# Ycblue/TransMIL-DeepGraft

Measured on AMD Instinct MI355X. Metric: slides/sec (fwd+bwd) at N=8192 patches, d=512, higher is better.
Workload: dtype bf16; 1 GPU; TransMIL_feat 2-class, 1 bag N=8192x512 per GPU, train step fwd+CE+bwd+allreduce+Lookahead(RAdam); execution=hipGraph replay of the whole step (one graph per resident bag), global_batch=1, seq_len=8192, parallelism=dp1, accumulate_grad_batches=1

## Files before the change

### include/transmil_hip.h

```cpp
#ifndef TRANSMIL_HIP_H
#define TRANSMIL_HIP_H
#include <stdint.h>

#ifdef __cplusplus
extern "C" {
#endif

const char* tm_last_error(void);
const char* tm_build_info(void);

enum { TM_EPI_PLAIN = 0, TM_EPI_QKV = 1, TM_EPI_SPLITK = 2 };
typedef struct tm_gemm_args {
  int M, N, K;
  int lda, ldb, ldc;
  int a_trans, b_kn;
  int ab_dtype, c_dtype;
  int splits, k_per_split;
  int mode;
  float alpha;
  const float* bias;
  int gelu;
  void* pre;
  int ld_pre;
  float drop_p, drop_scale;
  uint64_t seed;
  const float* resid;
  int accumulate;
  int grp_in, skip, grp_out, out_off, dup_n, dup_off;
  int nbags, nh, dh, seq;
  float qscale;
  const uint64_t* seed_ptr;
  float* colsum;
  int pre_bf16;
  int slab_bf16;
} tm_gemm_args;

int tm_gemm(const void* A, const void* B, void* C, const tm_gemm_args* args, void* stream);
typedef struct tm_reduce_queue tm_reduce_queue;
tm_reduce_queue* tm_reduce_queue_create(void);
void tm_reduce_queue_destroy(tm_reduce_queue* rq);
int tm_reduce_queue_pending(const tm_reduce_queue* rq);
int tm_reduce_flush(tm_reduce_queue* rq, void* stream);
int tm_splitk_reduce(const float* slab, float* out, int splits, long long count, float alpha,
                     int accumulate, tm_reduce_queue* rq, void* stream);
int tm_splitk_reduce_bf16(const void* slab, float* out, int splits, long long count, float alpha,
                          int accumulate, tm_reduce_queue* rq, void* stream);
long long tm_colsum_workspace(int rows, int cols, int rows_per_chunk);
int tm_colsum(const void* X, int dtype, int rows, int cols, int ld, int rows_per_chunk,
              float* work, float* out, int accumulate, tm_reduce_queue* rq, void* stream);

int tm_layernorm_fwd(const float* x, const float* gamma, const float* beta, float eps, int rows, int D,
                     int S, int n_pad, int pad, int dtype, void* y, float* mean, float* rstd, void* stream);
long long tm_layernorm_bwd_workspace(int rows, int D, int rows_per_block);
int tm_layernorm_bwd(const void* dy, int dtype, const float* x, const float* gamma, const float* mean,
                     const float* rstd, int rows, int D, int S, int n_pad, int pad, int rows_per_block,
                     int resid_cls_only, float* dx_accum, float* work, float* dgamma, float* dbeta,
                     tm_reduce_queue* rq, void* stream);
int tm_layernorm_bwd_seg(const void* dy, int dtype, const float* x, const float* gamma, const float* mean,
                         const float* rstd, int rows, int D, int S, int n_pad, int pad, int rows_per_block,
                         int resid_cls_only, const float* seg_add, int seg_len, int nseg, int seg_rows,
                         float* dx_accum, float* work, float* dgamma, float* dbeta, tm_reduce_queue* rq,
                         void* stream);
int tm_head_fwd(const float* h, int B, int S, int D, const float* gamma, const float* beta, float eps,
                const float* W, const float* bias, int C, float* logits, float* xhat, float* rstd,
                void* stream);
int tm_head_bwd(const float* dlogits, int B, int C, int S, int D, const float* xhat, const float* rstd,
                const float* gamma, const float* beta, const float* W, float* dW, float* dbias,
                float* dgamma, float* dbeta, float* dh, void* stream);
int tm_head_ce_fwd(const float* h, int B, int S, int D, const float* gamma, const float* beta, float eps,
                   const float* W, const float* bias, int C, const long long* label, float* logits, float* xhat,
// ... 258 lines not shown
```

### transmil_deepgraft_amd/_lib.py

```python
from __future__ import annotations

import ctypes as C
import os

_HERE = os.path.dirname(os.path.abspath(__file__))
LIB_PATH = os.environ.get("TRANSMIL_HIP_LIB", os.path.join(_HERE, "libtransmil_hip.so"))

F32, BF16 = 0, 1
EPI_PLAIN, EPI_QKV, EPI_SPLITK = 0, 1, 2

P = C.c_void_p
I = C.c_int
L = C.c_longlong
Fl = C.c_float
U64 = C.c_uint64


class GemmArgs(C.Structure):
    _fields_ = [("M", I), ("N", I), ("K", I), ("lda", I), ("ldb", I), ("ldc", I),
                ("a_trans", I), ("b_kn", I), ("ab_dtype", I), ("c_dtype", I),
                ("splits", I), ("k_per_split", I), ("mode", I), ("alpha", Fl),
                ("bias", P), ("gelu", I), ("pre", P), ("ld_pre", I),
                ("drop_p", Fl), ("drop_scale", Fl), ("seed", U64), ("resid", P),
                ("accumulate", I), ("grp_in", I), ("skip", I), ("grp_out", I),
# ... 4 lines not shown
class BmmJob(C.Structure):
    _fields_ = [("A", P), ("B", P), ("ta", I), ("tb", I), ("lda", I), ("ldb", I), ("sa", L), ("sb", L),
                ("A2", P), ("B2", P), ("ta2", I), ("tb2", I), ("lda2", I), ("ldb2", I), ("sa2", L), ("sb2", L),
                ("E1", P), ("e1", Fl), ("E2", P), ("e2", Fl), ("alpha", Fl), ("diag", Fl),
                ("C", P), ("ldc", I), ("sc", L), ("M", I), ("N", I), ("K", I),
                ("C2", P), ("c2_alpha", Fl), ("c2_diag", Fl), ("c2_e1", Fl),
                ("Ct", P), ("ct_plane", L), ("ct_mode", I), ("ct_reserved", I), ("Rd", P), ("Rw", P)]


OPTIM_MAX_TENSORS = 40


class OptimTensor(C.Structure):
    _fields_ = [("param", P), ("grad", P), ("numel", L), ("lr", Fl), ("weight_decay", Fl)]


class OptimTable(C.Structure):
    _fields_ = [("count", I), ("reserved", I), ("offset", L * (OPTIM_MAX_TENSORS + 1)),
                ("t", OptimTensor * OPTIM_MAX_TENSORS), ("hyper", P)]


CAST_MAX = 8


class CastTable(C.Structure):
    _fields_ = [("count", I), ("reserved", I), ("src", P * CAST_MAX), ("dst", P * CAST_MAX),
                ("offset", L * (CAST_MAX + 1))]


_SIGS = {
    "tm_last_error": (C.c_char_p, []),
    "tm_build_info": (C.c_char_p, []),
    "tm_gemm": (I, [P, P, P, C.POINTER(GemmArgs), P]),
    "tm_splitk_reduce": (I, [P, P, I, L, Fl, I, P, P]),
    "tm_splitk_reduce_bf16": (I, [P, P, I, L, Fl, I, P, P]),
    "tm_colsum_workspace": (L, [I, I, I]),
    "tm_colsum": (I, [P, I, I, I, I, I, P, P, I, P, P]),
    "tm_layernorm_fwd": (I, [P, P, P, Fl, I, I, I, I, I, I, P, P, P, P]),
    "tm_layernorm_bwd_workspace": (L, [I, I, I]),
    "tm_layernorm_bwd": (I, [P, I, P, P, P, P, I, I, I, I, I, I, I, P, P, P, P, P, P]),
    "tm_layernorm_bwd_seg": (I, [P, I, P, P, P, P, I, I, I, I, I, I, I, P, I, I, I, P, P, P, P, P, P]),
    "tm_head_fwd": (I, [P, I, I, I, P, P, Fl, P, P, I, P, P, P, P]),
    "tm_head_bwd": (I, [P, I, I, I, I, P, P, P, P, P, P, P, P, P, P, P]),
    "tm_head_ce_fwd": (I, [P, I, I, I, P, P, Fl, P, P, I, P, P, P, P, P, P, P, P, P]),
    "tm_head_ce_bwd": (I, [P, P, P, P, I, I, I, I, P, P, P, P, P, P, P, P, P, P, P, P]),
    "tm_nys_landmarks": (I, [I, P, P, I, I, P, P, P, P, P]),
    "tm_nys_sim2_softmax": (I, [P, P, I, P, P]),
    "tm_softmax_bwd_rows256": (I, [P, P, P, I, P]),
    "tm_nys_a3_workspace": (L, [I, I]),
    "tm_nys_a3_partials": (L, [I, I]),
    "tm_nys_a3_fwd": (I, [I, P, P, P, I, I, P, P, P, P]),
    "tm_nys_a3_fwd_sim2": (I, [P, P, P, P, I, I, P, P, P, P]),
    "tm_nys_a1_fwd": (I, [I, P, P, P, P, P, I, I, I, P, P, P]),
    "tm_cast_f32": (I, [I, P, P, L, P]),
    "tm_nys_conv_bwd_workspace": (L, [I, I, I]),
    "tm_nys_conv_bwd": (I, [I, P, P, P, P, I, I, I, P, P, P, P, P, P]),
    "tm_nys_a1_bwd_workspace": (L, [I, I, I]),
    "tm_nys_a1_bwd": (I, [I, P, P, P, P, P, P, I, I, I, I, P, P, P, P, I, P, P]),
    "tm_nys_a1_bwd_dqkv": (I, [P, P, P, P, P, P, I, I, I, P, Fl, P, P, P, P, P]),
    "tm_nys_a3_bwd_workspace": (L, [I, I]),
    "tm_nys_a3_bwd": (I, [I, P, P, P, P, P, P, I, I, I, P, P, P, P, I, P, P]),
    "tm_nys_assemble_dqkv": (I, [I, P, P, P, P, P, I, I, I, Fl, P, P]),
    "tm_nys_a3_bwd_fused": (I, [P, P, P, P, P, P, I, I, I, P, I, I, P, P, P, P, P, P]),
    "tm_nys_a3_bwd_slabs": (I, [I, I]),
    "tm_nys_assemble_q_slab": (I, [I, P, I, P, P, I, I, I, I, Fl, P, P]),
    "tm_nys_assemble_q_slab_inplace": (I, [P, P, I, I, I, I, Fl, P, P]),
# ... 143 lines not shown
```

### transmil_deepgraft_amd/csrc/gemm.hip

```cpp
#include <new>

#include "common.h"

#include <type_traits>
#include "../../include/transmil_hip.h"

namespace {

constexpr int BM = 128, BN = 128;
constexpr int EP_ROW = BN + 8;

template <typename T> struct Tile {
  static constexpr int E = 16 / sizeof(T);
  static constexpr int BK = 128 / sizeof(T);
  static constexpr int KROW = BK + E;
  static constexpr int TROW = BM + 32;
  static constexpr int KSTEPS = BK / 16;
  static constexpr int CHUNKS = BM * BK / E / 256;
};

template <typename T> union Chunk { f32x4 raw; T e[16 / sizeof(T)]; };

template <typename T>
TM_DEV void load_rows_full(Chunk<T> (&st)[Tile<T>::CHUNKS], const T* X, int ld, int r0, int k0, int tid) {
// ... 509 lines not shown
  auto mm = [](f32x16& c, const bf16x8& a, const bf16x8& b) { mma16(c, a, b); };
  bf16x8 a[2], b[2][2];
  rd_frag<A_KS, 0>(a[0], abase, akc); rd_frag<B_KS, 0>(b[0][0], b0, bkc0); rd_frag<B_KS, 0>(b[0][1], b1, bkc1);
  rd_frag<A_KS, 1>(a[1], abase, akc); rd_frag<B_KS, 1>(b[1][0], b0, bkc0); rd_frag<B_KS, 1>(b[1][1], b1, bkc1);
  wait_lgkm<RS>();
  mm(acc[0], a[0], b[0][0]);
  mm(acc[1], a[0], b[0][1]);
  rd_frag<A_KS, 2>(a[0], abase, akc); rd_frag<B_KS, 2>(b[0][0], b0, bkc0); rd_frag<B_KS, 2>(b[0][1], b1, bkc1);
  wait_lgkm<RS>();
  mm(acc[0], a[1], b[1][0]);
  mm(acc[1], a[1], b[1][1]);
  rd_frag<A_KS, 3>(a[1], abase, akc); rd_frag<B_KS, 3>(b[1][0], b0, bkc0); rd_frag<B_KS, 3>(b[1][1], b1, bkc1);
  wait_lgkm<RS>();
  mm(acc[0], a[0], b[0][0]);
  mm(acc[1], a[0], b[0][1]);
  wait_lgkm<0>();
  mm(acc[0], a[1], b[1][0]);
  mm(acc[1], a[1], b[1][1]);
}

__device__ unsigned long long g_gemm_stamps[2048 * 8];
template <bool ON>
TM_DEV void ring_stamp(unsigned long long (&ts)[8], int slot, bool real = false) {
  if constexpr (ON) {
    __builtin_amdgcn_sched_barrier(0);
    unsigned long long t;
    if (real) asm volatile("s_memrealtime %0\n\ts_waitcnt lgkmcnt(0)" : "=s"(t)::"memory");
    else asm volatile("s_memtime %0\n\ts_waitcnt lgkmcnt(0)" : "=s"(t)::"memory");
    __builtin_amdgcn_sched_barrier(0);
    ts[slot] = t;
  }
}

template <typename OutT, bool A_T, bool B_KN, bool STAMP = false, int KIND = EK_ANY>
__global__ __launch_bounds__(512) __attribute__((amdgpu_waves_per_eu(4))) void gemm_ring_kernel(const bf16* __restrict__ A, const bf16* __restrict__ B,
                                                        OutT* __restrict__ C, tm_gemm_args g) {
  extern __shared__ __attribute__((aligned(16))) char smem[];
  unsigned long long ts[8] = {0, 0, 0, 0, 0, 0, 0, 0};
  ring_stamp<STAMP>(ts, 0, true);
  ring_stamp<STAMP>(ts, 1);
  const int tid = threadIdx.x, lane = tid & 63;
  const int wave = __builtin_amdgcn_readfirstlane(tid >> 6);
  const int wm = wave >> 1, wn = wave & 1;
  int m0, n0, zs;
  tile_split_of_block(m0, n0, zs);
  const int kbeg = zs * g.k_per_split;
  const int kend = min(g.K, kbeg + g.k_per_split);
  const int nk = kend > kbeg ? (kend - kbeg) / 64 : 0;

  f32x16 acc[2];
  acc[0] = (f32x16){};
  acc[1] = (f32x16){};
  constexpr bool COLSUM = A_T && KIND == EK_SPLITK && !STAMP;
  const bool do_cs = COLSUM && g.colsum != nullptr && n0 == 0;
  const int cs_c = tid & 15, cs_r = tid >> 4;
  float csum[8] = {0.f, 0.f, 0.f, 0.f, 0.f, 0.f, 0.f, 0.f};
  unsigned akc[4] = {0, 0, 0, 0}, bkc0[4] = {0, 0, 0, 0}, bkc1[4] = {0, 0, 0, 0};
  unsigned aks = 0, bks0 = 0, bks1 = 0;
  if constexpr (A_T) aks = ks_addr(wm * 32, lane); else kc_addrs(akc, wm * 32, lane);
  if constexpr (B_KN) {
    bks0 = ks_addr(wn * 64, lane) + STAGE_BYTES / 2;
    bks1 = ks_addr(wn * 64 + 32, lane) + STAGE_BYTES / 2;
  } else {
    kc_addrs(bkc0, wn * 64, lane);
    kc_addrs(bkc1, wn * 64 + 32, lane);
#pragma unroll
    for (int s = 0; s < 4; ++s) { bkc0[s] += STAGE_BYTES / 2; bkc1[s] += STAGE_BYTES / 2; }
  }
  const unsigned ring = lds_u32(smem);

  auto issue = [&](int kt) {
    char* st = smem + (kt % NSTAGE) * STAGE_BYTES;
    const int k0 = kbeg + kt * 64;
    glds_tile<A_T>(st, A, g.lda, m0, g.M, k0, wave, lane);
    glds_tile<B_KN>(st + STAGE_BYTES / 2, B, g.ldb, n0, g.N, k0, wave, lane);
  };
#pragma unroll
  for (int t = 0; t < NSTAGE - 1; ++t)
// ... 34 lines not shown
    if (do_cs) {
#pragma unroll
      for (int e = 0; e < 8; ++e) {
        csum[e] += __shfl_xor(csum[e], 16, 64);
        csum[e] += __shfl_xor(csum[e], 32, 64);
      }
      __syncthreads();
      float* red = (float*)smem;
      if (lane < 16) {
#pragma unroll
        for (int e = 0; e < 8; ++e) red[wave * 128 + cs_c * 8 + e] = csum[e];
      }
      __syncthreads();
      if (tid < 128 && m0 + tid < g.M) {
        float s = 0.f;
#pragma unroll
        for (int w = 0; w < 8; ++w) s += red[w * 128 + tid];
        g.colsum[(size_t)zs * g.M + m0 + tid] = s;
      }
    }
  }
  if constexpr (STAMP) {
    ring_stamp<STAMP>(ts, 5);
    asm volatile("s_waitcnt vmcnt(0)" ::: "memory");
    ring_stamp<STAMP>(ts, 6);
    ring_stamp<STAMP>(ts, 7, true);
    const int blk = (blockIdx.z * gridDim.y + blockIdx.y) * gridDim.x + blockIdx.x;
    if (tid < 8 && blk < 2048) {
      unsigned long long v = ts[0];
#pragma unroll
      for (int i = 1; i < 8; ++i) v = tid == i ? ts[i] : v;
      g_gemm_stamps[blk * 8 + tid] = v;
    }
  }
}

constexpr int BM160 = 160;
constexpr int R160_A = BM160 * 128, R160_STAGE = R160_A + 128 * 128;

TM_DEV void tile160_of_block(int& m0, int& n0) {
  const int ntx = gridDim.x, nwg = gridDim.x * gridDim.y;
  const int orig = blockIdx.y * ntx + blockIdx.x;
  const int q = nwg / 8, r = nwg % 8, xcd = orig % 8;
  const int id = (xcd < r ? xcd * (q + 1) : r * (q + 1) + (xcd - r) * q) + orig / 8;
  m0 = (id / ntx) * BM160;
  n0 = (id % ntx) * BN;
}

template <typename OutT, bool B_KN, int KIND = EK_ANY>
__global__ __launch_bounds__(640) void gemm_ring160_kernel(const bf16* __restrict__ A, const bf16* __restrict__ B,
                                                           OutT* __restrict__ C, tm_gemm_args g) {
  extern __shared__ __attribute__((aligned(16))) char smem[];
  typedef __attribute__((address_space(3))) void lds_t;
  typedef __attribute__((address_space(1))) void glb_t;
  const int tid = threadIdx.x, lane = tid & 63;
  const int wave = __builtin_amdgcn_readfirstlane(tid >> 6);
  const int wm = wave >> 1, wn = wave & 1;
  int m0, n0;
  tile160_of_block(m0, n0);
  const int nk = g.K / 64;

  f32x16 acc[2];
  acc[0] = (f32x16){};
  acc[1] = (f32x16){};
  unsigned akc[4], bkc0[4] = {0, 0, 0, 0}, bkc1[4] = {0, 0, 0, 0};
  unsigned bks0 = 0, bks1 = 0;
// ... 385 lines not shown
      float t = slab[i];
      for (int z = 1; z < splits; ++z) t += slab[(size_t)z * count + i];
      t *= alpha;
      if (accumulate) t += out[i];
      out[i] = t;
    }
  }
}

template <typename T>
__global__ void colsum_partial_kernel(const T* __restrict__ X, int rows, int cols, int ld, int rows_per_chunk,
                                      float* __restrict__ part) {
  const int c = blockIdx.x * 64 + (threadIdx.x & 63);
  const int sub = threadIdx.x >> 6;
  const int r0 = blockIdx.y * rows_per_chunk, r1 = min(rows, r0 + rows_per_chunk);
  __shared__ float red[4][64];
  float s = 0.f;
  if (c < cols) {
    float p8[8] = {0.f, 0.f, 0.f, 0.f, 0.f, 0.f, 0.f, 0.f};
    int r = r0 + sub;
    for (; r + 28 < r1; r += 32) {
#pragma unroll
      for (int j = 0; j < 8; ++j) p8[j] += to_f(X[(size_t)(r + 4 * j) * ld + c]);
    }
    for (; r < r1; r += 4) p8[0] += to_f(X[(size_t)r * ld + c]);
    s = ((p8[0] + p8[1]) + (p8[2] + p8[3])) + ((p8[4] + p8[5]) + (p8[6] + p8[7]));
  }
  red[sub][threadIdx.x & 63] = s;
  __syncthreads();
  if (sub == 0 && c < cols)
    part[(size_t)blockIdx.y * cols + c] = red[0][threadIdx.x] + red[1][threadIdx.x] + red[2][threadIdx.x] + red[3][threadIdx.x];
}

}

extern "C" int tm_gemm(const void* A, const void* B, void* C, const tm_gemm_args* g, void* stream) {
  TM_REQUIRE(g && A && B && C, "gemm: null argument");
  TM_REQUIRE(g->M >= 0 && g->N >= 0 && g->K >= 0 && g->splits >= 1, "gemm: bad shape");
  TM_REQUIRE(g->mode != TM_EPI_SPLITK || g->c_dtype == TM_F32, "gemm: split-K slabs are fp32 (or bf16 via slab_bf16)");
  TM_REQUIRE(!g->slab_bf16 || (g->mode == TM_EPI_SPLITK && g->ab_dtype == TM_BF16),
             "gemm: slab_bf16 is for bf16 split-K weight gradients");
  TM_REQUIRE(g->k_per_split > 0, "gemm: k_per_split must be > 0");
  TM_REQUIRE(((uintptr_t)A % 16) == 0 && ((uintptr_t)B % 16) == 0, "gemm: operands must be 16-B aligned");
  const int E = g->ab_dtype == TM_BF16 ? 8 : 4;
  TM_REQUIRE(g->lda % E == 0 && g->ldb % E == 0, "gemm: leading dimensions must be multiples of 16 B");
  TM_REQUIRE(g->mode != TM_EPI_QKV || (g->dh % 8 == 0 && g->N % 8 == 0), "gemm: QKV scatter needs dh % 8 == 0");
  if (g->M == 0 || g->N == 0) return 0;
  TM_REQUIRE(!g->colsum || (g->ab_dtype == TM_BF16 && g->c_dtype == TM_F32 && g->a_trans && g->mode == TM_EPI_SPLITK &&
                            pick_path(*g) == PATH_RING && GEMM_SEL != GEMM_STAMP_RING),
             "gemm: colsum needs the bf16 split-K weight-gradient ring path (a_trans, K % 64 == 0, M % 8 == 0)");
  hipStream_t st = (hipStream_t)stream;
  if (g->ab_dtype == TM_BF16) {
    TM_REQUIRE(g->k_per_split % 64 == 0 || g->splits == 1, "gemm: bf16 k_per_split must be a multiple of 64");
    if (g->c_dtype == TM_BF16) return launch_t<bf16, bf16>(A, B, C, *g, st);
    return launch_t<bf16, float>(A, B, C, *g, st);
  }
  TM_REQUIRE(g->ab_dtype == TM_F32, "gemm: ab_dtype");
  TM_REQUIRE(g->k_per_split % 32 == 0 || g->splits == 1, "gemm: f32 k_per_split must be a multiple of 32");
  if (g->c_dtype == TM_BF16) return launch_t<float, bf16>(A, B, C, *g, st);
  return launch_t<float, float>(A, B, C, *g, st);
}

#ifdef TM_DIAG
extern "C" void tm_debug_set_gemm_sel(int sel) { g_gemm_sel = sel; }

extern "C" int tm_debug_gemm_stamps(unsigned long long* host, int count) {
  TM_REQUIRE(count > 0 && count <= 2048 * 8, "gemm_stamps: bad count");
  if (hipMemcpyFromSymbol(host, HIP_SYMBOL(g_gemm_stamps), count * sizeof(unsigned long long)) != hipSuccess) {
    tm_set_error("gemm_stamps: copy");
    return 1;
  }
  return 0;
}
#endif

namespace {
constexpr int DEFER_MAX = 48;
struct ReduceEntry {
  const void* slab;
  float* out;
  long long count;
  int splits;
  int accumulate;
  float alpha;
  int vec;
  int par;
  int bf16;
};
struct ReduceTable {
  ReduceEntry e[DEFER_MAX];
  long long off[DEFER_MAX + 1];
  int boff[DEFER_MAX + 1];
  int n;
// ... 229 lines not shown
```

### transmil_deepgraft_amd/engine.py

```python
from __future__ import annotations

import ctypes as C
import math
from dataclasses import dataclass

import torch

from . import _lib
from ._lib import BF16, F32, EPI_PLAIN, EPI_QKV, EPI_SPLITK, GemmArgs, BmmJob

NL = 256
DH = 64
TAPS = 33
PINV_ITERS = 6
LN_EPS = 1e-5
GEOMETRIES = ((DH, NL), (32, 128), (48, 192))
QROWS = NL + 32
CLS_Q_ROWS = True


class _Probe:

    def __init__(self):
        self.target = None
# ... 245 lines not shown
    def __exit__(self, *exc):
        try:
            if exc[0] is None and self.q.pending() > 0:
                self.q.flush()
        finally:
            _TLS.queue = self.prev
            self.q.close()
        return False


def _rq():
    q = getattr(_TLS, "queue", None)
    if q is not None and getattr(_TLS, "deferring", False):
        return q.handle
    return C.c_void_p(0)


class defer_reductions:

    def __enter__(self):
        self.prev = getattr(_TLS, "deferring", False)
        _TLS.deferring = getattr(_TLS, "queue", None) is not None
        return self

    def __exit__(self, *exc):
        _TLS.deferring = self.prev
        return False


def flush_reductions():
    q = getattr(_TLS, "queue", None)
    if q is not None:
        q.flush()


def nystrom_core_forward(qkv, geo: Geometry, wconv, tdtype, dt_code, pool, cls_row=None):
    if (geo.dh, geo.nl) != (DH, NL):
        if cls_row is not None:
            raise NotImplementedError("the class-row layer runs at dim_head=64, num_landmarks=256 only")
        return _nysg_core_forward(qkv, geo, wconv, pool)
    n, nbh, nh = geo.n, geo.nbh, geo.heads
    q, k, v = qkv[0], qkv[1], qkv[2]
    st = _stream()
    ql = pool(nbh * NL * DH).view(nbh, NL, DH)
    kl = pool(nbh * NL * DH).view(nbh, NL, DH)
    ql_t = pool(nbh * NL * DH, tdtype).view(nbh, NL, DH)
    kl_t = pool(nbh * NL * DH, tdtype).view(nbh, NL, DH)
    with probe("landmarks"):
        _lib.call("tm_nys_landmarks", dt_code, _p(q), _p(k), nbh, n, _p(ql), _p(kl), _p(ql_t), _p(kl_t), st)
    a2 = pool(nbh * NL * NL).view(nbh, NL, NL)
    w = pool(nbh * NL * DH).view(nbh, NL, DH)
    lse3 = pool(nbh * NL)
    work = pool(_lib.query("tm_nys_a3_workspace", nbh, n) // 4)
    prec = 1 if dt_code == BF16 else 0
    a2s = None
    if prec:
        a2s = pool(nbh * NL * NL)
        with probe("a3_fwd"):
            _lib.call("tm_nys_a3_fwd_sim2", _p(ql), _p(kl), _p(k), _p(v), nbh, n, _p(work), _p(a2), _p(a2s), st)
    else:
        with probe("a3_fwd"):
            _lib.call("tm_nys_a3_fwd", dt_code, _p(ql), _p(k), _p(v), nbh, n, _p(work), _p(w), _p(lse3), st)
    if prec:
        saved = pool(_lib.query("tm_pinv_split_saved_floats", nbh, PINV_ITERS))
        with probe("pinv_fwd"):
            _lib.call("tm_pinv_fwd_split_a3", _p(a2), _p(a2s), nbh, PINV_ITERS, _p(saved), _p(work),
# ... 220 lines not shown
    _lib.call("tm_nysg_assemble_dqkv", dh, nl, dt_code, _p(dq), _p(dql), _p(dk), _p(dkl), _p(dv), geo.B, nh, n,
              C.c_float(scale), _p(dqkv), st)
    return dqkv


def translayer_forward(H, geo: Geometry, prm, tdtype, dt_code, pool, drop_p, seed, seed_dev=None, cls_only=False):
    B, S, n, D, pad = geo.B, geo.S, geo.n, geo.D, geo.pad
    st = _stream()
    xn = pool(B * n * D, tdtype).view(B, n, D)
    mean = pool(B * S)
    rstd = pool(B * S)
    with probe("ln_fwd"):
        _lib.call("tm_layernorm_fwd", _p(H), _p(prm["norm_w"]), _p(prm["norm_b"]), C.c_float(LN_EPS), B * S, D,
                  S, n, pad, dt_code, _p(xn), _p(mean), _p(rstd), st)
    qkv = pool(3 * geo.nbh * n * DH, tdtype).view(3, geo.nbh, n, DH)
    with probe("qkv_gemm"):
        gemm(xn, prm["wqkv"], qkv, B * n, 3 * D, D, lda=D, ldb=D, ldc=0, dtype=dt_code,
             qkv=(B, geo.heads, DH, n, DH ** -0.5))
    merged, state = nystrom_core_forward(qkv, geo, prm["wconv"], tdtype, dt_code, pool,
                                         cls_row=pad if cls_only else None)
    Hout = pool(B * S * D).view(B * S, D)
    if cls_only:
        _lib.call("tm_cls_out_fwd", dt_code, _p(merged), _p(prm["wo"]), _p(prm["bo"]), _p(H), B, n, pad, S, D,
                  C.c_float(drop_p), C.c_uint64(seed), _p(seed_dev), _p(Hout), st)
    else:
        with probe("out_gemm"):
            gemm(merged, prm["wo"], Hout, B * n, D, D, lda=D, ldb=D, ldc=D, dtype=dt_code, c_dtype=F32,
                 bias=prm["bo"], drop_p=drop_p, seed=seed, seed_ptr=seed_dev, resid=H, rowmap=(n, pad, S, 0, 0, 0))
    saved = dict(xn=xn, mean=mean, rstd=rstd, qkv=qkv, merged=merged, core=state, seed=seed, seed_dev=seed_dev,
                 drop_p=drop_p, cls_only=cls_only)
    return Hout, saved


def translayer_backward(dH, H_in, saved, geo: Geometry, prm, grads, tdtype, dt_code, pool, dout=None, head=None):
    B, S, n, D, pad = geo.B, geo.S, geo.n, geo.D, geo.pad
    st = _stream()
    if saved["cls_only"]:
        dmerged = pool(B * D, tdtype).view(B, D)
        if head is not None:
            _lib.call("tm_cls_head_out_bwd", dt_code, *head, _p(dH), _p(saved["merged"]), _p(prm["wo"]), n, pad, S,
                      D, C.c_float(saved["drop_p"]), C.c_uint64(saved["seed"]), _p(saved["seed_dev"]),
                      _p(grads["wo"]), _p(grads["bo"]), _p(dmerged), st)
        else:
            _lib.call("tm_cls_out_bwd", dt_code, _p(dH), _p(saved["merged"]), _p(prm["wo"]), B, n, pad, S, D,
                      C.c_float(saved["drop_p"]), C.c_uint64(saved["seed"]), _p(saved["seed_dev"]), _p(grads["wo"]),
                      _p(grads["bo"]), _p(dmerged), st)
    else:
        if dout is None:
            dout = pool(B * n * D, tdtype).view(B, n, D)
            _lib.call("tm_dropout_bwd_pad", dt_code, _p(dH), B, S, n, pad, D, C.c_float(saved["drop_p"]),
                      C.c_uint64(saved["seed"]), _p(saved["seed_dev"]), _p(dout), st)
        with defer_reductions(), probe("wgrad_out"):
            weight_grad(dout, saved["merged"], grads["wo"], D, D, B * n, ldy=D, ldx=D, dtype=dt_code,
                        work_pool=pool, bias_out=grads["bo"])
        dmerged = pool(B * n * D, tdtype).view(B, n, D)
        with probe("dmerged_gemm"):
            gemm(dout, prm["wo"], dmerged, B * n, D, D, lda=D, ldb=D, ldc=D, b_kn=1, dtype=dt_code)
    qrows_on = (CLS_Q_ROWS and saved["cls_only"] and dt_code == BF16 and saved["core"]["a2s"] is not None
                and "wqkv_f32" in prm)
    dqkv, qrows = nystrom_core_backward(dmerged, saved["merged"], saved["qkv"], saved["core"], geo, prm["wconv"],
                                        tdtype, dt_code, pool, grads["wconv"], DH ** -0.5,
                                        cls_row=pad if saved["cls_only"] else None,
                                        xn=saved["xn"] if qrows_on else None)
    dxn = pool(B * n * D, tdtype).view(B, n, D)
    rpb = _LN_BWD_RPB
    if qrows is None:
        with defer_reductions(), probe("wgrad_qkv"):
            weight_grad(dqkv, saved["xn"], grads["wqkv"], 3 * D, D, B * n, ldy=3 * D, ldx=D, dtype=dt_code,
                        work_pool=pool)
        with probe("dxn_gemm"):
            gemm(dqkv, prm["wqkv"], dxn, B * n, D, 3 * D, lda=3 * D, ldb=D, ldc=D, b_kn=1, dtype=dt_code)
        with defer_reductions():
            work = pool(_lib.query("tm_layernorm_bwd_workspace", B * S, D, rpb) // 4)
            _lib.call("tm_layernorm_bwd", _p(dxn), dt_code, _p(H_in), _p(prm["norm_w"]), _p(saved["mean"]),
                      _p(saved["rstd"]), B * S, D, S, n, pad, rpb, int(saved["cls_only"]), _p(dH), _p(work),
                      _p(grads["norm_w"]),
                      _p(grads["norm_b"]), _rq(), st)
        return
    dkv = dqkv.view(B * n, 3 * D)[:, D:]
    with defer_reductions(), probe("wgrad_qkv"):
        weight_grad(dkv, saved["xn"], grads["wqkv"][D:], 2 * D, D, B * n, ldy=3 * D, ldx=D, dtype=dt_code,
                    work_pool=pool)
    with probe("dxn_gemm"):
        gemm(dkv, prm["wqkv"][D:], dxn, B * n, D, 2 * D, lda=3 * D, ldb=D, ldc=D, b_kn=1, dtype=dt_code)
    Aq, Xs = qrows
    scale = DH ** -0.5
    wq = prm["wqkv_f32"][:D]
    gwq = grads["wqkv"][:D]
    G = pool(B * QROWS * D).view(B, QROWS, D)
    with probe("cls_q_products"):
        jobs = [bmm_job(Aq.view(B * QROWS, D), 0, wq, 0, G.view(B * QROWS, D), B * QROWS, D, D, alpha=scale),
                bmm_job(Aq[0], 1, Xs[0], 0, gwq, D, D, QROWS, alpha=scale)]
        bmm(jobs, 1, 1)
        for b in range(1, B):
            bmm([bmm_job(Aq[b], 1, Xs[b], 0, gwq, D, D, QROWS, alpha=scale, E1=gwq, e1=1.0)], 1, 1)
    with defer_reductions():
        work = pool(_lib.query("tm_layernorm_bwd_workspace", B * S, D, rpb) // 4)
        _lib.call("tm_layernorm_bwd_seg", _p(dxn), dt_code, _p(H_in), _p(prm["norm_w"]), _p(saved["mean"]),
                  _p(saved["rstd"]), B * S, D, S, n, pad, rpb, int(saved["cls_only"]), _p(G), n // NL, NL, QROWS,
                  _p(dH), _p(work), _p(grads["norm_w"]), _p(grads["norm_b"]), _rq(), st)


FC1_PLAIN = {"main": "_fc1.0", "inner": None}
FC1_RCC2048 = {"main": "_fc1.3", "inner": ("_fc1.0", "_fc1.2")}
FC1_EMBED = {"main": None, "inner": None}


class TransMILEngine:

    def __init__(self, dtype: torch.dtype = torch.bfloat16, fc1=None, head="_fc", cls_only=True):
        if dtype not in (torch.bfloat16, torch.float32):
            raise ValueError("compute dtype must be torch.bfloat16 or torch.float32")
        self.tdtype = dtype
        self.dt_code = BF16 if dtype == torch.bfloat16 else F32
        self.fc1 = FC1_PLAIN if fc1 is None else fc1
        self.head = head
        self.cls_only = cls_only
        _lib.lib()

    def _cast(self, w, pool):
        if self.dt_code == F32:
            return w.contiguous()
        out = pool(w.numel(), self.tdtype)
        _lib.call("tm_cast_f32", self.dt_code, _p(w.contiguous()), _p(out), w.numel(), _stream())
        return out.view(w.shape)

    def _cast_many(self, ws, pool):
        ws = [w.contiguous() for w in ws]
        if self.dt_code == F32:
            return ws
        tab = _lib.CastTable()
        tab.count = len(ws)
        outs = []
        off = 0
        for i, w in enumerate(ws):
            o = pool(w.numel(), self.tdtype).view(w.shape)
            tab.src[i], tab.dst[i], tab.offset[i] = w.data_ptr(), o.data_ptr(), off
            off += w.numel()
            outs.append(o)
        tab.offset[len(ws)] = off
        _lib.call("tm_cast_f32_many", self.dt_code, C.byref(tab), _stream())
# ... 139 lines not shown
        B, N, F, D, S = geo.B, geo.N, geo.F, geo.D, geo.S
        st = _stream()
        g = out if out is not None else {name: torch.empty_like(p, dtype=torch.float32)
                                         for name, p in params.items()}
        Ccls = prm["fc_w"].shape[0]
        dH = (torch.empty if self.cls_only else torch.zeros)(B * S, D, dtype=torch.float32, device=dev)
        head = None
        if gloss is not None and dlogits is None and self.cls_only and B == 1 and Ccls <= 4 and D == 512:
            gls = gloss.float().contiguous()
            ctx["_gloss"] = gls
            head = (_p(ctx["ce"][1]), _p(ctx["ce"][0]), _p(gls), Ccls, _p(ctx["xhat"]), _p(ctx["hrstd"]),
                    _p(prm["norm_w"]), _p(prm["norm_b"]), _p(prm["fc_w"]), _p(g[self.head + ".weight"]),
                    _p(g[self.head + ".bias"]), _p(g["norm.weight"]), _p(g["norm.bias"]))
        elif gloss is not None:
            label, prob = ctx["ce"][0], ctx["ce"][1]
            scratch = None if (B == 1 and Ccls <= 4) else pool(B * Ccls)
            dl_in = None if dlogits is None else dlogits.float().contiguous()
            _lib.call("tm_head_ce_bwd", _p(prob), _p(label), _p(gloss.float().contiguous()), _p(dl_in), B, Ccls, S,
                      D, _p(ctx["xhat"]), _p(ctx["hrstd"]), _p(prm["norm_w"]), _p(prm["norm_b"]), _p(prm["fc_w"]),
                      _p(g[self.head + ".weight"]), _p(g[self.head + ".bias"]), _p(g["norm.weight"]),
                      _p(g["norm.bias"]), _p(dH), _p(scratch), st)
        else:
            _lib.call("tm_head_bwd", _p(dlogits.contiguous()), B, Ccls, S, D, _p(ctx["xhat"]), _p(ctx["hrstd"]),
                      _p(prm["norm_w"]), _p(prm["norm_b"]), _p(prm["fc_w"]), _p(g[self.head + ".weight"]),
                      _p(g[self.head + ".bias"]),
                      _p(g["norm.weight"]), _p(g["norm.bias"]), _p(dH), st)
        dout1 = None
        for li, Hin, saved in ((2, ctx["H2"], ctx["s2"]), (1, ctx["H0"], ctx["s1"])):
            pre = f"layer{li}."
            gl = {"wo": g[pre + "attn.to_out.0.weight"], "bo": g[pre + "attn.to_out.0.bias"],
                  "wqkv": g[pre + "attn.to_qkv.weight"], "wconv": g[pre + "attn.res_conv.weight"],
                  "norm_w": g[pre + "norm.weight"], "norm_b": g[pre + "norm.bias"]}
            translayer_backward(dH, Hin, saved, geo, prm[li], gl, self.tdtype, self.dt_code, pool, dout=dout1,
                                head=head if li == 2 else None)
            if li == 2:
                dH1 = pool(B * S * D).view(B * S, D)
                work = pool(_lib.query("tm_ppeg_bwd_workspace", B, geo.G, D) // 4)
                s1 = ctx["s1"]
                dout1 = pool(B * geo.n * D, self.tdtype).view(B, geo.n, D)
                with probe("ppeg_bwd"), defer_reductions():
                    _lib.call("tm_ppeg_bwd", _p(ctx["H1"]), _p(dH), B, geo.G, D, _p(prm["wfold"]), _p(dH1),
                              _p(work), _p(g["pos_layer.proj.weight"]), _p(g["pos_layer.proj.bias"]),
                              _p(g["pos_layer.proj1.weight"]), _p(g["pos_layer.proj1.bias"]),
                              _p(g["pos_layer.proj2.weight"]), _p(g["pos_layer.proj2.bias"]), self.dt_code,
                              _p(dout1), geo.n, geo.pad, C.c_float(s1["drop_p"]), C.c_uint64(s1["seed"]),
                              _p(s1["seed_dev"]), _rq(), st)
                dH = dH1
                flush_reductions()
                if ready is not None:
                    ready(0)
            elif ready is not None and parts >= 3 and self.fc1["main"] is not None:
                flush_reductions()
                ready(1)
        if self.fc1["main"] is None:
            dHv = dH.view(B, S, D)
            dx = dHv[:, 1:N + 1].clone()
            if geo.add:
                dx[:, :geo.add] += dHv[:, N + 1:]
            torch.sum(dHv[:, 0], dim=0, out=g["cls_token"].view(D))
            g["__dx__"] = dx
            flush_reductions()
            if ready is not None:
                ready(1)
            return g
        dpre = pool(B * N * D, self.tdtype).view(B * N, D)
        _lib.call("tm_fc1_gelu_bwd", self.dt_code, _p(dH), _p(ctx["pre"]), B, N, S, geo.add, D, _p(dpre),
                  _p(g["cls_token"]), st)
# ... 106 lines not shown
```

Baseline: 901.3 slides/sec.

## Fuse backward weight-grad and data-grad GEMMs into one paired grid launch

Adds a pair mode in which the split-K weight-gradient GEMM and the plain data-gradient GEMM of the out-projection and QKV backward are captured and launched as a single kernel, with workgroups assigned to either GEMM in XCD-contiguous order. The aim is to fill the device with both small GEMMs at once instead of running two under-occupied launches back to back, and to cut one launch boundary. The cost is extra host bookkeeping through thread-local state, and co-scheduled tiles may compete for cache and LDS.

```diff
diff --git a/include/transmil_hip.h b/include/transmil_hip.h
--- a/include/transmil_hip.h
+++ b/include/transmil_hip.h
@@ -36,6 +36,8 @@
 } tm_gemm_args;
 
 int tm_gemm(const void* A, const void* B, void* C, const tm_gemm_args* args, void* stream);
+int tm_gemm_pair_begin(void* stream);
+int tm_gemm_pair_end(void* stream);
 typedef struct tm_reduce_queue tm_reduce_queue;
 tm_reduce_queue* tm_reduce_queue_create(void);
 void tm_reduce_queue_destroy(tm_reduce_queue* rq);
diff --git a/transmil_deepgraft_amd/_lib.py b/transmil_deepgraft_amd/_lib.py
--- a/transmil_deepgraft_amd/_lib.py
+++ b/transmil_deepgraft_amd/_lib.py
@@ -60,6 +60,8 @@
     "tm_last_error": (C.c_char_p, []),
     "tm_build_info": (C.c_char_p, []),
     "tm_gemm": (I, [P, P, P, C.POINTER(GemmArgs), P]),
+    "tm_gemm_pair_begin": (I, [P]),
+    "tm_gemm_pair_end": (I, [P]),
     "tm_splitk_reduce": (I, [P, P, I, L, Fl, I, P, P]),
     "tm_splitk_reduce_bf16": (I, [P, P, I, L, Fl, I, P, P]),
     "tm_colsum_workspace": (L, [I, I, I]),
diff --git a/transmil_deepgraft_amd/csrc/gemm.hip b/transmil_deepgraft_amd/csrc/gemm.hip
--- a/transmil_deepgraft_amd/csrc/gemm.hip
+++ b/transmil_deepgraft_amd/csrc/gemm.hip
@@ -565,18 +565,16 @@
   }
 }
 
-template <typename OutT, bool A_T, bool B_KN, bool STAMP = false, int KIND = EK_ANY>
-__global__ __launch_bounds__(512) __attribute__((amdgpu_waves_per_eu(4))) void gemm_ring_kernel(const bf16* __restrict__ A, const bf16* __restrict__ B,
-                                                        OutT* __restrict__ C, tm_gemm_args g) {
+template <typename OutT, bool A_T, bool B_KN, bool STAMP, int KIND>
+TM_DEV void gemm_ring_tile(const bf16* A, const bf16* B, OutT* C, const tm_gemm_args& g, const int tid,
+                           const int m0, const int n0, const int zs) {
   extern __shared__ __attribute__((aligned(16))) char smem[];
   unsigned long long ts[8] = {0, 0, 0, 0, 0, 0, 0, 0};
   ring_stamp<STAMP>(ts, 0, true);
   ring_stamp<STAMP>(ts, 1);
-  const int tid = threadIdx.x, lane = tid & 63;
+  const int lane = tid & 63;
   const int wave = __builtin_amdgcn_readfirstlane(tid >> 6);
   const int wm = wave >> 1, wn = wave & 1;
-  int m0, n0, zs;
-  tile_split_of_block(m0, n0, zs);
   const int kbeg = zs * g.k_per_split;
   const int kend = min(g.K, kbeg + g.k_per_split);
   const int nk = kend > kbeg ? (kend - kbeg) / 64 : 0;
@@ -677,6 +675,57 @@
       for (int i = 1; i < 8; ++i) v = tid == i ? ts[i] : v;
       g_gemm_stamps[blk * 8 + tid] = v;
     }
+  }
+}
+
+template <typename OutT, bool A_T, bool B_KN, bool STAMP = false, int KIND = EK_ANY>
+__global__ __launch_bounds__(512) __attribute__((amdgpu_waves_per_eu(4))) void gemm_ring_kernel(const bf16* __restrict__ A, const bf16* __restrict__ B,
+                                                        OutT* __restrict__ C, tm_gemm_args g) {
+  int m0, n0, zs;
+  tile_split_of_block(m0, n0, zs);
+  gemm_ring_tile<OutT, A_T, B_KN, STAMP, KIND>(A, B, C, g, threadIdx.x, m0, n0, zs);
+}
+
+enum { PAIR_INTERLEAVED = 0, PAIR_W_FIRST = 1 };
+struct PairGrid {
+  int nw, nd;
+  int gw, gd;
+  int ntx_w, per_w;
+  int ntx_d;
+};
+
+TM_DEV int xcd_contiguous_id(int orig, int nwg) {
+  const int q = nwg / 8, r = nwg % 8, xcd = orig % 8;
+  return (xcd < r ? xcd * (q + 1) : r * (q + 1) + (xcd - r) * q) + orig / 8;
+}
+
+template <int ORDER>
+__global__ __launch_bounds__(512) __attribute__((amdgpu_waves_per_eu(4))) void gemm_ring_pair_kernel(
+    const bf16* __restrict__ Aw, const bf16* __restrict__ Bw, float* __restrict__ Cw, tm_gemm_args gw,
+    const bf16* __restrict__ Ad, const bf16* __restrict__ Bd, bf16* __restrict__ Cd, tm_gemm_args gd, PairGrid p) {
+  const int grp = blockIdx.x >> 3, x = blockIdx.x & 7;
+  const int groups = p.gw + p.gd;
+  int wbefore, is_w;
+  if (ORDER == PAIR_W_FIRST) {
+    wbefore = min(grp, p.gw);
+    is_w = grp < p.gw;
+  } else {
+    wbefore = (int)((long long)grp * p.gw / groups);
+    is_w = (int)((long long)(grp + 1) * p.gw / groups) > wbefore;
+  }
+  if (is_w) {
+    const int orig = wbefore * 8 + x;
+    if (orig >= p.nw) return;
+    const int id = xcd_contiguous_id(orig, p.nw);
+    const int zs = id / p.per_w, rr = id - zs * p.per_w;
+    gemm_ring_tile<float, true, true, false, EK_SPLITK>(Aw, Bw, Cw, gw, threadIdx.x, (rr / p.ntx_w) * BM,
+                                                        (rr % p.ntx_w) * BN, zs);
+  } else {
+    const int orig = (grp - wbefore) * 8 + x;
+    if (orig >= p.nd) return;
+    const int id = xcd_contiguous_id(orig, p.nd);
+    gemm_ring_tile<bf16, false, true, false, EK_PLAIN>(Ad, Bd, Cd, gd, threadIdx.x, (id / p.ntx_d) * BM,
+                                                       (id % p.ntx_d) * BN, 0);
   }
 }
 
@@ -1128,9 +1177,52 @@
     part[(size_t)blockIdx.y * cols + c] = red[0][threadIdx.x] + red[1][threadIdx.x] + red[2][threadIdx.x] + red[3][threadIdx.x];
 }
 
-}
-
-extern "C" int tm_gemm(const void* A, const void* B, void* C, const tm_gemm_args* g, void* stream) {
+struct HeldGemm {
+  const void* A;
+  const void* B;
+  void* C;
+  tm_gemm_args g;
+};
+struct PairState {
+  bool open = false;
+  void* stream = nullptr;
+  int n = 0;
+  HeldGemm h[2];
+};
+thread_local PairState t_pair;
+
+constexpr int PAIR_ORDER = PAIR_W_FIRST;
+
+inline bool pair_w_ok(const tm_gemm_args& g) {
+  return g.ab_dtype == TM_BF16 && g.c_dtype == TM_F32 && g.a_trans == 1 && g.b_kn == 1 && g.mode == TM_EPI_SPLITK &&
+         ring_ok(g);
+}
+inline bool pair_d_ok(const tm_gemm_args& g) {
+  return g.ab_dtype == TM_BF16 && g.c_dtype == TM_BF16 && g.a_trans == 0 && g.b_kn == 1 && g.splits == 1 &&
+         epilogue_kind(g) == EK_PLAIN && ring_ok(g);
+}
+
+int launch_pair(const HeldGemm& w, const HeldGemm& d, hipStream_t st) {
+  PairGrid p;
+  p.ntx_w = (w.g.N + BN - 1) / BN;
+  p.per_w = p.ntx_w * ((w.g.M + BM - 1) / BM);
+  p.nw = p.per_w * w.g.splits;
+  p.ntx_d = (d.g.N + BN - 1) / BN;
+  p.nd = p.ntx_d * ((d.g.M + BM - 1) / BM);
+  p.gw = (p.nw + 7) / 8;
+  p.gd = (p.nd + 7) / 8;
+  constexpr size_t epi = (size_t)BM * EP_ROW * sizeof(float);
+  constexpr size_t lds = RING_BYTES > epi ? RING_BYTES : epi;
+  auto kernel = gemm_ring_pair_kernel<PAIR_ORDER>;
+  tm_allow_smem(kernel, lds);
+  kernel<<<dim3((unsigned)(p.gw + p.gd) * 8), 512, lds, st>>>((const bf16*)w.A, (const bf16*)w.B, (float*)w.C, w.g,
+                                                               (const bf16*)d.A, (const bf16*)d.B, (bf16*)d.C, d.g, p);
+  TM_CHECK_LAUNCH();
+  return 0;
+}
+
+int gemm_check(const void* A, const void* B, void* C, const tm_gemm_args* g, bool* empty) {
+  *empty = false;
   TM_REQUIRE(g && A && B && C, "gemm: null argument");
   TM_REQUIRE(g->M >= 0 && g->N >= 0 && g->K >= 0 && g->splits >= 1, "gemm: bad shape");
   TM_REQUIRE(g->mode != TM_EPI_SPLITK || g->c_dtype == TM_F32, "gemm: split-K slabs are fp32 (or bf16 via slab_bf16)");
@@ -1141,20 +1233,81 @@
   const int E = g->ab_dtype == TM_BF16 ? 8 : 4;
   TM_REQUIRE(g->lda % E == 0 && g->ldb % E == 0, "gemm: leading dimensions must be multiples of 16 B");
   TM_REQUIRE(g->mode != TM_EPI_QKV || (g->dh % 8 == 0 && g->N % 8 == 0), "gemm: QKV scatter needs dh % 8 == 0");
-  if (g->M == 0 || g->N == 0) return 0;
+  if (g->M == 0 || g->N == 0) {
+    *empty = true;
+    return 0;
+  }
   TM_REQUIRE(!g->colsum || (g->ab_dtype == TM_BF16 && g->c_dtype == TM_F32 && g->a_trans && g->mode == TM_EPI_SPLITK &&
                             pick_path(*g) == PATH_RING && GEMM_SEL != GEMM_STAMP_RING),
              "gemm: colsum needs the bf16 split-K weight-gradient ring path (a_trans, K % 64 == 0, M % 8 == 0)");
-  hipStream_t st = (hipStream_t)stream;
   if (g->ab_dtype == TM_BF16) {
     TM_REQUIRE(g->k_per_split % 64 == 0 || g->splits == 1, "gemm: bf16 k_per_split must be a multiple of 64");
-    if (g->c_dtype == TM_BF16) return launch_t<bf16, bf16>(A, B, C, *g, st);
-    return launch_t<bf16, float>(A, B, C, *g, st);
+    return 0;
   }
   TM_REQUIRE(g->ab_dtype == TM_F32, "gemm: ab_dtype");
   TM_REQUIRE(g->k_per_split % 32 == 0 || g->splits == 1, "gemm: f32 k_per_split must be a multiple of 32");
-  if (g->c_dtype == TM_BF16) return launch_t<float, bf16>(A, B, C, *g, st);
-  return launch_t<float, float>(A, B, C, *g, st);
+  return 0;
+}
+
+int gemm_launch(const void* A, const void* B, void* C, const tm_gemm_args& g, hipStream_t st) {
+  if (g.ab_dtype == TM_BF16) {
+    if (g.c_dtype == TM_BF16) return launch_t<bf16, bf16>(A, B, C, g, st);
+    return launch_t<bf16, float>(A, B, C, g, st);
+  }
+  if (g.c_dtype == TM_BF16) return launch_t<float, bf16>(A, B, C, g, st);
+  return launch_t<float, float>(A, B, C, g, st);
+}
+
+}
+
+extern "C" int tm_gemm(const void* A, const void* B, void* C, const tm_gemm_args* g, void* stream) {
+  PairState& ps = t_pair;
+  const bool hold = ps.open && ps.stream == stream;
+  bool empty;
+  const int rc = gemm_check(A, B, C, g, &empty);
+  if (rc != 0) {
+    if (hold) ps = PairState();
+    return rc;
+  }
+  if (empty) return 0;
+  if (!hold) return gemm_launch(A, B, C, *g, (hipStream_t)stream);
+  if (ps.n == 2) {
+    ps = PairState();
+    tm_set_error("gemm: more than two calls between tm_gemm_pair_begin and tm_gemm_pair_end");
+    return 1;
+  }
+  ps.h[ps.n++] = HeldGemm{A, B, C, *g};
+  return 0;
+}
+
+extern "C" int tm_gemm_pair_begin(void* stream) {
+  PairState& ps = t_pair;
+  if (ps.open) {
+    ps = PairState();
+    tm_set_error("gemm_pair_begin: a pair is already open on this thread");
+    return 1;
+  }
+  ps.open = true;
+  ps.stream = stream;
+  ps.n = 0;
+  return 0;
+}
+
+extern "C" int tm_gemm_pair_end(void* stream) {
+  const PairState ps = t_pair;
+  if (!ps.open) return 0;
+  t_pair = PairState();
+  TM_REQUIRE(ps.stream == stream, "gemm_pair_end: not the stream of tm_gemm_pair_begin");
+  hipStream_t st = (hipStream_t)stream;
+  if (ps.n == 2 && GEMM_SEL == GEMM_AUTO) {
+    if (pair_w_ok(ps.h[0].g) && pair_d_ok(ps.h[1].g)) return launch_pair(ps.h[0], ps.h[1], st);
+    if (pair_d_ok(ps.h[0].g) && pair_w_ok(ps.h[1].g)) return launch_pair(ps.h[1], ps.h[0], st);
+  }
+  for (int i = 0; i < ps.n; ++i) {
+    const int rc = gemm_launch(ps.h[i].A, ps.h[i].B, ps.h[i].C, ps.h[i].g, st);
+    if (rc != 0) return rc;
+  }
+  return 0;
 }
 
 #ifdef TM_DIAG
diff --git a/transmil_deepgraft_amd/engine.py b/transmil_deepgraft_amd/engine.py
--- a/transmil_deepgraft_amd/engine.py
+++ b/transmil_deepgraft_amd/engine.py
@@ -301,6 +301,29 @@
     q = getattr(_TLS, "queue", None)
     if q is not None:
         q.flush()
+
+
+PAIR_SITES = ("out", "qkv")
+
+
+class gemm_pair:
+
+    def __init__(self, on=True):
+        self.on = bool(on) and getattr(probe, "target", None) is None and getattr(_TLS, "queue", None) is not None
+
+    def __enter__(self):
+        if self.on:
+            _lib.call("tm_gemm_pair_begin", _stream())
+        return self
+
+    def __exit__(self, *exc):
+        if self.on:
+            try:
+                _lib.call("tm_gemm_pair_end", _stream())
+            except RuntimeError:
+                if exc[0] is None:
+                    raise
+        return False
 
 
 def nystrom_core_forward(qkv, geo: Geometry, wconv, tdtype, dt_code, pool, cls_row=None):
@@ -587,9 +610,13 @@
     return Hout, saved
 
 
-def translayer_backward(dH, H_in, saved, geo: Geometry, prm, grads, tdtype, dt_code, pool, dout=None, head=None):
+def translayer_backward(dH, H_in, saved, geo: Geometry, prm, grads, tdtype, dt_code, pool, dout=None, head=None,
+                        pair_gemms=False):
     B, S, n, D, pad = geo.B, geo.S, geo.n, geo.D, geo.pad
     st = _stream()
+    on = dt_code == BF16 and (geo.dh, geo.nl) == (DH, NL)
+    names = PAIR_SITES if pair_gemms is True else (pair_gemms or ())
+    pair_out, pair_qkv, pair_kv = (on and k in names for k in ("out", "qkv", "kv"))
     if saved["cls_only"]:
         dmerged = pool(B * D, tdtype).view(B, D)
         if head is not None:
@@ -605,12 +632,13 @@
             dout = pool(B * n * D, tdtype).view(B, n, D)
             _lib.call("tm_dropout_bwd_pad", dt_code, _p(dH), B, S, n, pad, D, C.c_float(saved["drop_p"]),
                       C.c_uint64(saved["seed"]), _p(saved["seed_dev"]), _p(dout), st)
-        with defer_reductions(), probe("wgrad_out"):
-            weight_grad(dout, saved["merged"], grads["wo"], D, D, B * n, ldy=D, ldx=D, dtype=dt_code,
-                        work_pool=pool, bias_out=grads["bo"])
         dmerged = pool(B * n * D, tdtype).view(B, n, D)
-        with probe("dmerged_gemm"):
-            gemm(dout, prm["wo"], dmerged, B * n, D, D, lda=D, ldb=D, ldc=D, b_kn=1, dtype=dt_code)
+        with gemm_pair(pair_out):
+            with defer_reductions(), probe("wgrad_out"):
+                weight_grad(dout, saved["merged"], grads["wo"], D, D, B * n, ldy=D, ldx=D, dtype=dt_code,
+                            work_pool=pool, bias_out=grads["bo"])
+            with probe("dmerged_gemm"):
+                gemm(dout, prm["wo"], dmerged, B * n, D, D, lda=D, ldb=D, ldc=D, b_kn=1, dtype=dt_code)
     qrows_on = (CLS_Q_ROWS and saved["cls_only"] and dt_code == BF16 and saved["core"]["a2s"] is not None
                 and "wqkv_f32" in prm)
     dqkv, qrows = nystrom_core_backward(dmerged, saved["merged"], saved["qkv"], saved["core"], geo, prm["wconv"],
@@ -620,11 +648,12 @@
     dxn = pool(B * n * D, tdtype).view(B, n, D)
     rpb = _LN_BWD_RPB
     if qrows is None:
-        with defer_reductions(), probe("wgrad_qkv"):
-            weight_grad(dqkv, saved["xn"], grads["wqkv"], 3 * D, D, B * n, ldy=3 * D, ldx=D, dtype=dt_code,
-                        work_pool=pool)
-        with probe("dxn_gemm"):
-            gemm(dqkv, prm["wqkv"], dxn, B * n, D, 3 * D, lda=3 * D, ldb=D, ldc=D, b_kn=1, dtype=dt_code)
+        with gemm_pair(pair_qkv):
+            with defer_reductions(), probe("wgrad_qkv"):
+                weight_grad(dqkv, saved["xn"], grads["wqkv"], 3 * D, D, B * n, ldy=3 * D, ldx=D, dtype=dt_code,
+                            work_pool=pool)
+            with probe("dxn_gemm"):
+                gemm(dqkv, prm["wqkv"], dxn, B * n, D, 3 * D, lda=3 * D, ldb=D, ldc=D, b_kn=1, dtype=dt_code)
         with defer_reductions():
             work = pool(_lib.query("tm_layernorm_bwd_workspace", B * S, D, rpb) // 4)
             _lib.call("tm_layernorm_bwd", _p(dxn), dt_code, _p(H_in), _p(prm["norm_w"]), _p(saved["mean"]),
@@ -633,11 +662,12 @@
                       _p(grads["norm_b"]), _rq(), st)
         return
     dkv = dqkv.view(B * n, 3 * D)[:, D:]
-    with defer_reductions(), probe("wgrad_qkv"):
-        weight_grad(dkv, saved["xn"], grads["wqkv"][D:], 2 * D, D, B * n, ldy=3 * D, ldx=D, dtype=dt_code,
-                    work_pool=pool)
-    with probe("dxn_gemm"):
-        gemm(dkv, prm["wqkv"][D:], dxn, B * n, D, 2 * D, lda=3 * D, ldb=D, ldc=D, b_kn=1, dtype=dt_code)
+    with gemm_pair(pair_kv):
+        with defer_reductions(), probe("wgrad_qkv"):
+            weight_grad(dkv, saved["xn"], grads["wqkv"][D:], 2 * D, D, B * n, ldy=3 * D, ldx=D, dtype=dt_code,
+                        work_pool=pool)
+        with probe("dxn_gemm"):
+            gemm(dkv, prm["wqkv"][D:], dxn, B * n, D, 2 * D, lda=3 * D, ldb=D, ldc=D, b_kn=1, dtype=dt_code)
     Aq, Xs = qrows
     scale = DH ** -0.5
     wq = prm["wqkv_f32"][:D]
@@ -662,6 +692,8 @@
 
 
 class TransMILEngine:
+
+    pair_gemms = True
 
     def __init__(self, dtype: torch.dtype = torch.bfloat16, fc1=None, head="_fc", cls_only=True):
         if dtype not in (torch.bfloat16, torch.float32):
@@ -867,7 +899,7 @@
                   "wqkv": g[pre + "attn.to_qkv.weight"], "wconv": g[pre + "attn.res_conv.weight"],
                   "norm_w": g[pre + "norm.weight"], "norm_b": g[pre + "norm.bias"]}
             translayer_backward(dH, Hin, saved, geo, prm[li], gl, self.tdtype, self.dt_code, pool, dout=dout1,
-                                head=head if li == 2 else None)
+                                head=head if li == 2 else None, pair_gemms=self.pair_gemms)
             if li == 2:
                 dH1 = pool(B * S * D).view(B * S, D)
                 work = pool(_lib.query("tm_ppeg_bwd_workspace", B, geo.G, D) // 4)
```

Result: faster. 922.1 slides/sec (median of 6 runs) (+2.3%).
